# thunlp/ConvDR

Measured on AMD Instinct MI355X. Metric: passages encoded/sec + query x passage IP-scored/sec, 768-d, higher is better.
Workload: dtype bf16

## Files before the change

### convdr_amd/csrc/encoder.hip

```cpp
#include "gemm_launch.hpp"
#include "gemm_ln.hpp"

#include "../../include/convdr_hip.h"

namespace convdr {

struct EncBufs {
  int32_t* status;
  int32_t *tok_id, *tok_pos;
  bf16_t *X, *Q, *K, *Vt, *ctx, *Hm, *cls_b, *cls_ctx, *cls_x, *cls_x1;
  float *Y, *cls_y, *cls_f, *head_y;
  float* slab;
  int64_t ldt;
  size_t total;
};

constexpr int64_t SPLITK_MAX_ROWS = 42 * 128;
constexpr int SPLITK_MAX_SPLIT = 4;
static int64_t g_ffn2_splitk = 1;

static EncBufs enc_plan(const convdr_encoder_config* c, int64_t rows, int B, char* base) {
  EncBufs p;
  size_t o = 0;
  auto take = [&](size_t bytes) { size_t at = o; o = align_up(o + bytes, 256); return (char*)((uintptr_t)base + at); };
  const int H = c->hidden, I = c->intermediate;
  const int64_t rs = rows + 128;
  p.ldt = align_up((size_t)rows + 64, 8);
  p.status = (int32_t*)take(256);
  p.tok_id = (int32_t*)take(rs * 4);
  p.tok_pos = (int32_t*)take(rs * 4);
  p.X = (bf16_t*)take(rs * H * 2);
  p.Q = (bf16_t*)take(rs * H * 2);
  p.K = (bf16_t*)take(rs * H * 2);
  p.Vt = (bf16_t*)take((size_t)H * p.ldt * 2);
  p.ctx = (bf16_t*)take(rs * H * 2);
  p.Hm = (bf16_t*)take(rs * I * 2);
  p.Y = (float*)take(rs * H * 4);
  p.slab = rows <= SPLITK_MAX_ROWS ? (float*)take((size_t)SPLITK_MAX_SPLIT * rs * H * 4) : nullptr;
  const int64_t Bp = B + 128;
  p.cls_b = (bf16_t*)take(Bp * H * 2);
  p.cls_ctx = (bf16_t*)take(Bp * H * 2);
  p.cls_x = (bf16_t*)take(Bp * H * 2);
  p.cls_x1 = (bf16_t*)take(Bp * H * 2);
  p.cls_y = (float*)take(Bp * H * 4);
  p.cls_f = (float*)take(Bp * H * 4);
  p.head_y = (float*)take(Bp * (c->out_dim > 0 ? c->out_dim : 1) * 4);
  p.total = o;
  return p;
}

static int64_t g_fused_ln_max_k = 1 << 30;
static int64_t g_hm_blocked = 1;
static int64_t g_fused_ln_min_rows = 128 * 192;

static bool fused_ln_applies(int64_t rows, int H, int K) {
  return H == 768 && rows >= g_fused_ln_min_rows && K % LN_SLICE == 0 && K <= g_fused_ln_max_k;
}
static int gemm_resid_ln(const bf16_t* W, const bf16_t* Wks, const bf16_t* A, int64_t rows, int H, int K, const float* bias,
                         const bf16_t* R, const float* gamma, const float* beta, float eps, float* Yf, bf16_t* X,
                         const char* name, hipStream_t st, bool a_blocked = false, float* slab = nullptr) {
  if (fused_ln_applies(rows, H, K)) {
    static DeviceOnce attr_done;
    if (attr_done.first())
      CONVDR_CHECK_HIP(
          hipFuncSetAttribute((const void*)k_gemm_resid_ln, hipFuncAttributeMaxDynamicSharedMemorySize, LN_SMEM_BYTES));
    GemmLnArgs a{W, A, rows, K, bias, R, gamma, beta, eps, X,
                 K == 768 ? (unsigned long long*)g_gemm_trace_ln : nullptr, Wks, a_blocked ? 1 : 0, 0};
#ifdef CONVDR_ENABLE_TRACE
    static const int dbg_epi = getenv("CONVDR_DBG_SKIP_EPI") ? atoi(getenv("CONVDR_DBG_SKIP_EPI")) : 0;
    a.dbg_skip_epi = dbg_epi == 1;
#endif
    ProfScope prof(name, st);
    hipLaunchKernelGGL(k_gemm_resid_ln, dim3((unsigned)ceil_div64(rows, TileLN::TL)), dim3(512), LN_SMEM_BYTES, st, a);
    CONVDR_CHECK_LAUNCH("k_gemm_resid_ln");
    return 0;
  }
  GemmArgs g{};
  int ns = 1;
  if (slab && g_ffn2_splitk && H == 768 && K >= 2048 && rows <= SPLITK_MAX_ROWS) {
    const int64_t tiles = ceil_div64(rows, 128) * (H / 128), slots = (int64_t)device_cu_count() * 2;
    for (int c = SPLITK_MAX_SPLIT; c >= 2; c >>= 1)
      if (tiles * c <= slots && K % (c * GEMM_BK) == 0) { ns = c; break; }
  }
  if (ns > 1) {
    g.rows = rows; g.W = W; g.X = A; g.N = H; g.K = K; g.k_split_len = K / ns; g.Cf = slab;
    if (int e = launch_gemm<EPI_SLAB_F32>(g, st, name)) return e;
    ProfScope prof("layernorm", st);
    hipLaunchKernelGGL(k_slab_finish_ln<3>, dim3((unsigned)ceil_div64(rows, 4)), dim3(256), 0, st, slab, ns, rows, bias, R, gamma, beta,
                       eps, X);
    CONVDR_CHECK_LAUNCH("k_slab_finish_ln");
    return 0;
  }
  g.rows = rows; g.W = W; g.X = A; g.N = H; g.K = K; g.bias = bias; g.Cf = Yf; g.R = R;
  if (int e = launch_gemm<EPI_RESID_F32>(g, st, name)) return e;
  ProfScope prof("layernorm", st);
  launch_layernorm_bf16(Yf, rows, H, gamma, beta, eps, X, st);
  CONVDR_CHECK_LAUNCH("k_layernorm");
  return 0;
}

static int check_config(const convdr_encoder_config* c) {
  CONVDR_REQUIRE(c->hidden % 128 == 0 && c->hidden <= 1024, "encoder: hidden must be a multiple of 128, <= 1024 (got %d)",
                 c->hidden);
  CONVDR_REQUIRE(c->heads * 64 == c->hidden, "encoder: head_dim must be 64 (hidden=%d heads=%d)", c->hidden, c->heads);
  CONVDR_REQUIRE(c->intermediate % 64 == 0, "encoder: intermediate %% 64 != 0 (%d)", c->intermediate);
  CONVDR_REQUIRE(c->out_dim == 0 || (c->out_dim % 4 == 0 && c->out_dim <= 1024), "encoder: bad out_dim %d", c->out_dim);
  return 0;
}

int encoder_layer_forward(const convdr_encoder_config* c, const convdr_layer_weights* w, const EncBufs& p,
                          const int32_t* cu, const int32_t* lens, int64_t rows, int B, int max_len, float* lse,
                          bool cls_only, hipStream_t st) {
  const int H = c->hidden, I = c->intermediate;
  GemmArgs g{};
  g.rows = rows;
  g.W = (const bf16_t*)w->wqkv; g.X = p.X; g.N = 3 * H; g.K = H; g.bias = w->bqkv;
  g.Qo = p.Q; g.Ko = p.K; g.Vt = p.Vt; g.H = H; g.ldt = p.ldt;
  const bf16_t *xin = p.X, *ctx = p.ctx;
  bf16_t* x1 = p.X;
  int64_t n = rows;
  const bool blk_on = g_hm_blocked != 0;
  const bool ctx_blocked = blk_on && !cls_only && fused_ln_applies(rows, H, H);
  const bool qk_blocked = blk_on && fused_ln_applies(rows, H, H);
  g.qk_blocked = qk_blocked ? 1 : 0;
  if (!cls_only) {
    if (int e = launch_gemm<EPI_QKV>(g, st, "gemm_qkv")) return e;
    AttnArgs a{p.Q, p.K, p.Vt, p.ldt, cu, lens, H, (int64_t)H, p.ctx, lse, 0.125f, (unsigned long long*)g_attn_trace};
    ProfScope prof("attention", st);
    if (ctx_blocked && qk_blocked) {
      hipLaunchKernelGGL((k_attention_fwd<false, true, true>), dim3((max_len + 127) / 128, c->heads, B), dim3(256), ATT_SMEM_BYTES, st, a);
    } else {
      hipLaunchKernelGGL(k_attention_fwd<false>, dim3((max_len + 127) / 128, c->heads, B), dim3(256), ATT_SMEM_BYTES, st, a);
    }
    CONVDR_CHECK_LAUNCH("k_attention_fwd");
  } else {
    hipLaunchKernelGGL(k_gather_cls, dim3((B + 3) / 4), dim3(256), 0, st, cu, B, H, p.X, (const float*)nullptr, p.cls_x,
                       (float*)nullptr);
    CONVDR_CHECK_LAUNCH("k_gather_cls");
    g.W = (const bf16_t*)w->wqkv + (size_t)H * H; g.bias = w->bqkv + H; g.N = 2 * H; g.third0 = 1;
    if (int e = launch_gemm<EPI_QKV>(g, st, "gemm_qkv")) return e;
    GemmArgs gq{};
    gq.rows = B; gq.W = (const bf16_t*)w->wqkv; gq.X = p.cls_x; gq.N = H; gq.K = H; gq.bias = w->bqkv; gq.Cb = p.Q;
    if (int e = launch_gemm<EPI_BF16>(gq, st, "gemm_qkv")) return e;
    AttnArgs a{p.Q, p.K, p.Vt, p.ldt, cu, lens, H, (int64_t)H, p.cls_ctx, nullptr, 0.125f, nullptr};
    ProfScope prof("attention", st);
    if (qk_blocked) hipLaunchKernelGGL((k_attention_fwd<true, false, true>), dim3(1, c->heads, B), dim3(256), ATT_SMEM_BYTES, st, a);
    else hipLaunchKernelGGL(k_attention_fwd<true>, dim3(1, c->heads, B), dim3(256), ATT_SMEM_BYTES, st, a);
    CONVDR_CHECK_LAUNCH("k_attention_fwd<cls>");
    xin = p.cls_x; ctx = p.cls_ctx; x1 = p.cls_x1; n = B;
  }
  if (int e = gemm_resid_ln((const bf16_t*)w->wo, (const bf16_t*)w->wo_ks, ctx, n, H, H, w->bo, xin, w->ln1_g, w->ln1_b, c->ln_eps, p.Y, x1,
                            "gemm_attn_out", st, ctx_blocked))
    return e;
  GemmArgs g2{};
  g2.rows = n; g2.W = (const bf16_t*)w->w1; g2.X = x1; g2.N = I; g2.K = H; g2.bias = w->b1; g2.Cb = p.Hm;
  const bool blocked = blk_on && !cls_only && fused_ln_applies(n, H, I) && I % 256 == 0 && (I / 256) * ceil_div64(n, 256) >= 192;
  if (blocked) {
    if (int e = launch_gemm<EPI_GELU_BLK>(g2, st, "gemm_ffn1")) return e;
    return gemm_resid_ln((const bf16_t*)w->w2, (const bf16_t*)w->w2_ks, p.Hm, n, H, I, w->b2, x1, w->ln2_g, w->ln2_b, c->ln_eps, p.Y,
                         p.X, "gemm_ffn2", st, true);
  }
  if (int e = launch_gemm<EPI_GELU_BF16>(g2, st, "gemm_ffn1")) return e;
  if (cls_only) {
    g2 = GemmArgs{};
    g2.rows = n; g2.W = (const bf16_t*)w->w2; g2.X = p.Hm; g2.N = H; g2.K = I; g2.bias = w->b2; g2.Cf = p.Y; g2.R = x1;
    return launch_gemm<EPI_RESID_F32>(g2, st, "gemm_ffn2");
  }
  return gemm_resid_ln((const bf16_t*)w->w2, (const bf16_t*)w->w2_ks, p.Hm, n, H, I, w->b2, x1, w->ln2_g, w->ln2_b, c->ln_eps, p.Y, p.X, "gemm_ffn2", st,
                       false, p.slab);
}

}

using namespace convdr;

extern "C" size_t convdr_encoder_workspace_bytes(const convdr_encoder_config* cfg, int64_t rows, int B) {
  return enc_plan(cfg, rows, B, nullptr).total;
}

extern "C" int convdr_cast_f32_bf16(const float* x, void* y, int64_t n, convdr_stream_t stream) {
  CONVDR_REQUIRE(n % 4 == 0, "convdr_cast_f32_bf16: n %% 4 != 0 (%lld)", (long long)n);
  if (n == 0) return 0;
  const int64_t n4 = n / 4;
  const unsigned grid = (unsigned)(ceil_div64(n4, 256) < 4096 ? ceil_div64(n4, 256) : 4096);
  hipLaunchKernelGGL(k_cast_f32_bf16, dim3(grid), dim3(256), 0, (hipStream_t)stream, x, (bf16_t*)y, n4);
  CONVDR_CHECK_LAUNCH("k_cast_f32_bf16");
  return 0;
}

extern "C" int convdr_encoder_forward(const convdr_encoder_config* cfg, const convdr_encoder_weights* w,
                                      const void* input_ids, int ids_are_int32, const int64_t* attention_mask, int B, int L,
                                      const int32_t* cu_seqlens, const int32_t* seq_lens, int64_t rows, int max_len,
                                      void* workspace, size_t workspace_bytes, float* out, convdr_stream_t stream) {
  hipStream_t st = (hipStream_t)stream;
  if (int e = check_config(cfg)) return e;
  CONVDR_REQUIRE(B > 0 && L > 0 && rows > 0 && rows % 8 == 0 && max_len > 0 && max_len <= L,
                 "convdr_encoder_forward: bad sizes B=%d L=%d rows=%lld max_len=%d", B, L, (long long)rows, max_len);
  const EncBufs p = enc_plan(cfg, rows, B, (char*)workspace);
  CONVDR_REQUIRE(workspace_bytes >= p.total, "convdr_encoder_forward: workspace too small (%zu < %zu)", workspace_bytes,
                 p.total);
  const int H = cfg->hidden;
  CONVDR_CHECK_HIP(hipMemset2DAsync(p.Vt + rows, p.ldt * 2, 0, (p.ldt - rows) * 2, H, st));
  CONVDR_CHECK_HIP(hipMemsetAsync(p.status, 0, 256, st));
  hipLaunchKernelGGL(k_seq_pack, dim3((B + 3) / 4), dim3(256), 0, st, input_ids, ids_are_int32, attention_mask, seq_lens, B, L, cu_seqlens,
                     cfg->kind, cfg->pad_idx, cfg->max_pos, cfg->vocab, p.tok_id, p.tok_pos, p.status);
  CONVDR_CHECK_LAUNCH("k_seq_pack");
  {
    ProfScope prof("embed_ln", st);
    hipLaunchKernelGGL(k_embed_ln, dim3((unsigned)ceil_div64(rows, 4)), dim3(256), 0, st, p.tok_id, p.tok_pos, rows, H,
                       w->word_emb, w->pos_emb, w->type_emb, w->emb_ln_g, w->emb_ln_b, cfg->ln_eps, p.X, DropSite{0u, 0u, 1.f});
    CONVDR_CHECK_LAUNCH("k_embed_ln");
  }
  for (int l = 0; l < cfg->layers; ++l) {
    const convdr_layer_weights* lw = &w->layers[l];
    const bool last = l + 1 == cfg->layers;
    if (int e = encoder_layer_forward(cfg, lw, p, cu_seqlens, seq_lens, rows, B, max_len, nullptr, last && !cfg->pool_mean, st))
      return e;
    if (last && cfg->pool_mean) {
      hipLaunchKernelGGL(k_masked_mean, dim3(B), dim3(256), 0, st, p.X, cu_seqlens, seq_lens, H, p.cls_b,
                         cfg->out_dim > 0 ? p.cls_f : out);
      CONVDR_CHECK_LAUNCH("k_masked_mean");
    } else if (last) {
      float* cls_out = cfg->out_dim > 0 ? p.cls_f : out;
      hipLaunchKernelGGL(k_layernorm, dim3((B + 3) / 4), dim3(256), 0, st, p.Y, (int64_t)B, H, lw->ln2_g, lw->ln2_b,
                         cfg->ln_eps, p.cls_b, cls_out);
      CONVDR_CHECK_LAUNCH("k_layernorm(cls)");
    }
  }
  if (cfg->out_dim > 0) {
    GemmArgs g{};
    g.rows = B; g.W = (const bf16_t*)w->head_w; g.X = p.cls_b; g.N = cfg->out_dim; g.K = H; g.bias = w->head_b;
    g.Cf = p.head_y;
    if (int e = launch_gemm<EPI_F32>(g, st, "gemm_head")) return e;
    hipLaunchKernelGGL(k_layernorm, dim3((B + 3) / 4), dim3(256), 0, st, p.head_y, (int64_t)B, cfg->out_dim,
                       w->head_ln_g, w->head_ln_b, cfg->head_ln_eps, (bf16_t*)nullptr, out);
    CONVDR_CHECK_LAUNCH("k_layernorm(head)");
  }
  return 0;
}

extern "C" int convdr_encoder_debug_layout(const convdr_encoder_config* cfg, int64_t rows, int B, int64_t* out) {
  const EncBufs p = enc_plan(cfg, rows, B, nullptr);
  const void* v[13] = {p.tok_id, p.tok_pos, p.X, p.Q, p.K, p.Vt, p.ctx, p.Hm, p.Y, p.cls_b, p.cls_y, p.cls_f, p.head_y};
  for (int i = 0; i < 13; ++i) out[i] = (int64_t)(size_t)v[i];
  out[13] = p.ldt;
  return 0;
}

namespace convdr {
static __global__ void __launch_bounds__(256) k_pack_kslice(const bf16_t* __restrict__ w, int n, int k, bf16_t* __restrict__ out) {
  const int64_t total = (int64_t)n * (k / 8);
  for (int64_t i = (int64_t)blockIdx.x * blockDim.x + threadIdx.x; i < total; i += (int64_t)gridDim.x * blockDim.x) {
    const int c = (int)(i & 3);
    const int64_t sr = i >> 2;
    const int r = (int)(sr % n), s = (int)(sr / n);
    *(uint4*)(out + i * 8) = *(const uint4*)(w + (int64_t)r * k + s * 32 + c * 8);
  }
}
}

extern "C" int convdr_pack_kslice(const void* w_bf16, int n, int k, void* out, convdr_stream_t stream) {
  CONVDR_REQUIRE(n > 0 && k > 0 && k % 32 == 0, "convdr_pack_kslice: bad shape %d x %d", n, k);
  const int64_t total = (int64_t)n * (k / 8);
  hipLaunchKernelGGL(k_pack_kslice, dim3((unsigned)(ceil_div64(total, 256) < 4096 ? ceil_div64(total, 256) : 4096)), dim3(256), 0,
                     (hipStream_t)stream, (const bf16_t*)w_bf16, n, k, (bf16_t*)out);
  CONVDR_CHECK_LAUNCH("k_pack_kslice");
  return 0;
}

extern "C" int convdr_set_option(const char* name, int64_t value) {
  if (strcmp(name, "fused_ln_min_rows") == 0) {
    g_fused_ln_min_rows = value;
    return 0;
  }
  if (strcmp(name, "hm_blocked") == 0) {
    g_hm_blocked = value;
    return 0;
  }
  if (strcmp(name, "gemm_tile_policy") == 0) {
    g_gemm_tile_policy = value;
    return 0;
  }
  if (strcmp(name, "attn_bwd_fused") == 0) {
    g_attn_bwd_fused = value;
    return 0;
  }
  if (strcmp(name, "embed_bwd_deterministic") == 0) {
    g_embed_bwd_det = value;
    return 0;
  }
  if (strcmp(name, "ip_fused_finish") == 0) {
    convdr::g_ip_fused_finish = value;
    return 0;
  }
  if (strcmp(name, "gelu_gp") == 0) {
    g_gelu_gp = value;
    return 0;
  }
  if (strcmp(name, "ffn2_splitk") == 0) {
    g_ffn2_splitk = value;
    return 0;
  }
  if (strcmp(name, "ln_rows") == 0) {
    g_ln_rows = value;
    return 0;
  }
  if (strcmp(name, "ln_bwd_rows") == 0) {
    g_ln_bwd_rows = value;
    return 0;
  }
  if (strcmp(name, "fused_ln_max_k") == 0) {
    g_fused_ln_max_k = value;
    return 0;
  }
  if (strcmp(name, "clock_probe") == 0) {
    g_clock_probe = (void*)(uintptr_t)value;
    g_clock_probe_next = 0;
    return 0;
  }
  if (strcmp(name, "clock_probe_slots") == 0) {
    g_clock_probe_slots = value > 0 ? value : 1;
    return 0;
  }
  if (strcmp(name, "attn_trace") == 0) {
    g_attn_trace = (void*)(uintptr_t)value;
    return 0;
  }
  if (strcmp(name, "gemm_trace_ln") == 0) {
    g_gemm_trace_ln = (void*)(uintptr_t)value;
    return 0;
  }
  if (strcmp(name, "gemm_trace") == 0) {
    g_gemm_trace = (void*)(uintptr_t)value;
    return 0;
  }
  set_error("convdr_set_option: unknown option %s", name);
  return -1;
}
```

Measured before the change: 44800.

## Fold K/V projections into CLS-only last-layer attention via query-weight algebra

```diff
diff --git a/convdr_amd/csrc/cls_fold.hpp b/convdr_amd/csrc/cls_fold.hpp
--- /dev/null
+++ b/convdr_amd/csrc/cls_fold.hpp
@@ -0,0 +1,261 @@
+#pragma once
+#include "gemm_nt.hpp"
+
+namespace convdr {
+
+union Frag8 {
+  bf16x8 v;
+  uint32_t u[4];
+  uint4 q;
+  uint2 d[2];
+};
+
+__device__ __forceinline__ void split_bf16x8(const float* x, Frag8& hi, Frag8& lo) {
+#pragma unroll
+  for (int i = 0; i < 4; ++i) {
+    const uint32_t h = pack_bf16x2(x[2 * i], x[2 * i + 1]);
+    hi.u[i] = h;
+    lo.u[i] = pack_bf16x2(x[2 * i] - __uint_as_float(h << 16), x[2 * i + 1] - __uint_as_float(h & 0xffff0000u));
+  }
+}
+
+constexpr int64_t CLS_FOLD_MIN_ROWS = 16384;
+constexpr int FOLD_ROWS = 64;
+constexpr int FOLD_NC = 128;
+constexpr int FOLD_LDW = FOLD_NC + 4;
+
+static __global__ void __launch_bounds__(256) k_cls_key_fold(const bf16_t* __restrict__ Q, const bf16_t* __restrict__ Wk, int B,
+                                                             int H, float scale, float* __restrict__ U) {
+  __shared__ __attribute__((aligned(16))) bf16_t ws[64 * FOLD_LDW];
+  const int tid = threadIdx.x, lane = tid & 63, wave = tid >> 6, lr = lane & 15, g = lane >> 4;
+  const int h = blockIdx.y, heads = H >> 6;
+  const int b = blockIdx.x * FOLD_ROWS + wave * 16 + lr;
+  const int bc = b < B ? b : B - 1;
+  Frag8 qf[2];
+#pragma unroll
+  for (int ks = 0; ks < 2; ++ks) qf[ks].q = *(const uint4*)(Q + (int64_t)bc * H + h * 64 + ks * 32 + g * 8);
+  const bf16_t* wk = Wk + (int64_t)h * 64 * H;
+  float* up = U + ((int64_t)bc * heads + h) * H;
+  for (int n0 = 0; n0 < H; n0 += FOLD_NC) {
+    __syncthreads();
+#pragma unroll
+    for (int i = 0; i < 4; ++i) {
+      const int idx = i * 256 + tid, r = idx >> 4, c = (idx & 15) * 8;
+      const uint4 v = *(const uint4*)(wk + (int64_t)r * H + n0 + c);
+      *(uint2*)(ws + r * FOLD_LDW + c) = make_uint2(v.x, v.y);
+      *(uint2*)(ws + r * FOLD_LDW + c + 4) = make_uint2(v.z, v.w);
+    }
+    __syncthreads();
+#pragma unroll 2
+    for (int nt = 0; nt < FOLD_NC / 16; ++nt) {
+      f32x4 acc = {0.f, 0.f, 0.f, 0.f};
+#pragma unroll
+      for (int ks = 0; ks < 2; ++ks) {
+        const bf16_t* wp = ws + (ks * 32 + g * 8) * FOLD_LDW + nt * 16 + lr;
+        Frag8 a;
+#pragma unroll
+        for (int i = 0; i < 4; ++i) a.u[i] = (uint32_t)wp[(2 * i) * FOLD_LDW] | ((uint32_t)wp[(2 * i + 1) * FOLD_LDW] << 16);
+        acc = __builtin_amdgcn_mfma_f32_16x16x32_bf16(a.v, qf[ks].v, acc, 0, 0, 0);
+      }
+      if (b < B) *(float4*)(up + n0 + nt * 16 + g * 4) = make_float4(scale * acc[0], scale * acc[1], scale * acc[2], scale * acc[3]);
+    }
+  }
+}
+
+static __global__ void __launch_bounds__(256) k_cls_value_fold(const float* __restrict__ Z, const bf16_t* __restrict__ Wv,
+                                                               const float* __restrict__ bv, int B, int H,
+                                                               bf16_t* __restrict__ ctx) {
+  const int tid = threadIdx.x, lane = tid & 63, wave = tid >> 6, lr = lane & 15, g = lane >> 4;
+  const int h = blockIdx.y, heads = H >> 6;
+  const int b = blockIdx.x * FOLD_ROWS + wave * 16 + lr;
+  const int bc = b < B ? b : B - 1;
+  const float* zp = Z + ((int64_t)bc * heads + h) * H + g * 8;
+  const bf16_t* wv = Wv + ((int64_t)h * 64 + lr) * H + g * 8;
+  f32x4 acc[4];
+#pragma unroll
+  for (int mt = 0; mt < 4; ++mt) acc[mt] = f32x4{0.f, 0.f, 0.f, 0.f};
+  for (int k0 = 0; k0 < H; k0 += 128) {
+    f32x4 z[8];
+#pragma unroll
+    for (int i = 0; i < 4; ++i) {
+      z[2 * i] = __builtin_nontemporal_load((const f32x4*)(zp + k0 + i * 32));
+      z[2 * i + 1] = __builtin_nontemporal_load((const f32x4*)(zp + k0 + i * 32 + 4));
+    }
+#pragma unroll
+    for (int i = 0; i < 4; ++i) {
+      const float x[8] = {z[2 * i][0], z[2 * i][1], z[2 * i][2], z[2 * i][3], z[2 * i + 1][0], z[2 * i + 1][1], z[2 * i + 1][2], z[2 * i + 1][3]};
+      Frag8 zh, zl;
+      split_bf16x8(x, zh, zl);
+#pragma unroll
+      for (int mt = 0; mt < 4; ++mt) {
+        Frag8 a;
+        a.q = *(const uint4*)(wv + (int64_t)mt * 16 * H + k0 + i * 32);
+        acc[mt] = __builtin_amdgcn_mfma_f32_16x16x32_bf16(a.v, zh.v, acc[mt], 0, 0, 0);
+        acc[mt] = __builtin_amdgcn_mfma_f32_16x16x32_bf16(a.v, zl.v, acc[mt], 0, 0, 0);
+      }
+    }
+  }
+  if (b >= B) return;
+#pragma unroll
+  for (int mt = 0; mt < 4; ++mt) {
+    const int j0 = h * 64 + mt * 16 + g * 4;
+    const float4 bias = *(const float4*)(bv + j0);
+    uint2 o;
+    o.x = pack_bf16x2(acc[mt][0] + bias.x, acc[mt][1] + bias.y);
+    o.y = pack_bf16x2(acc[mt][2] + bias.z, acc[mt][3] + bias.w);
+    *(uint2*)(ctx + (int64_t)b * H + j0) = o;
+  }
+}
+
+constexpr int POOL_T = 32;
+template <int HC>
+constexpr int pool_smem_bytes() { return POOL_T * (128 * HC + 4) * 2 + 4 * POOL_T * 16 * 4; }
+
+template <int HC>
+static __global__ void __launch_bounds__(256, HC <= 6 ? 2 : 1) k_cls_pool(const bf16_t* __restrict__ X, const float* __restrict__ U,
+                                                         const int32_t* __restrict__ cu, const int32_t* __restrict__ lens,
+                                                         float* __restrict__ Z) {
+  constexpr int H = 128 * HC, LDX = H + 4, HEADS = 2 * HC, NLD = H / 64, HQ = H / 4, RP = H / 8;
+  extern __shared__ __attribute__((aligned(16))) unsigned char pool_smem[];
+  bf16_t* xs = (bf16_t*)pool_smem;
+  float* sp = (float*)(pool_smem + POOL_T * LDX * 2);
+  const int tid = threadIdx.x, lane = tid & 63, wave = tid >> 6, lr = lane & 15, g = lane >> 4;
+  const int b = blockIdx.x;
+  const int64_t base = cu[b];
+  const int len = lens[b];
+  const int nchunks = (len + POOL_T - 1) / POOL_T;
+
+  u32x4_t pre[NLD];
+  auto fetch = [&](int c) {
+#pragma unroll
+    for (int i = 0; i < NLD; ++i) {
+      const int idx = i * 256 + tid, r = idx / RP, cs = idx % RP, t = c * POOL_T + r;
+      pre[i] = u32x4_t{0u, 0u, 0u, 0u};
+      if (t < len) pre[i] = __builtin_nontemporal_load((const u32x4_t*)(X + (base + t) * H + cs * 8));
+    }
+  };
+  auto stash = [&]() {
+#pragma unroll
+    for (int i = 0; i < NLD; ++i) {
+      const int idx = i * 256 + tid, r = idx / RP, cs = idx % RP;
+      *(uint2*)(xs + r * LDX + cs * 8) = make_uint2(pre[i][0], pre[i][1]);
+      *(uint2*)(xs + r * LDX + cs * 8 + 4) = make_uint2(pre[i][2], pre[i][3]);
+    }
+  };
+  fetch(0);
+
+  Frag8 uh[HC], ul[HC];
+  {
+    const float* up = U + ((int64_t)b * HEADS + (lr < HEADS ? lr : 0)) * H + wave * HQ + g * 8;
+#pragma unroll
+    for (int ks = 0; ks < HC; ++ks) {
+      const f32x4 u0 = __builtin_nontemporal_load((const f32x4*)(up + ks * 32));
+      const f32x4 u1 = __builtin_nontemporal_load((const f32x4*)(up + ks * 32 + 4));
+      const float m = lr < HEADS ? 1.f : 0.f;
+      const float x[8] = {m * u0[0], m * u0[1], m * u0[2], m * u0[3], m * u1[0], m * u1[1], m * u1[2], m * u1[3]};
+      split_bf16x8(x, uh[ks], ul[ks]);
+    }
+  }
+  f32x4 acc[NLD];
+#pragma unroll
+  for (int nt = 0; nt < NLD; ++nt) acc[nt] = f32x4{0.f, 0.f, 0.f, 0.f};
+  float m_run = -INFINITY, l_run = 0.f;
+
+  stash();
+  __syncthreads();
+  for (int c = 0; c < nchunks; ++c) {
+    if (c + 1 < nchunks) fetch(c + 1);
+#pragma unroll
+    for (int mt = 0; mt < 2; ++mt) {
+      f32x4 s = {0.f, 0.f, 0.f, 0.f};
+      const bf16_t* xp = xs + (mt * 16 + lr) * LDX + wave * HQ + g * 8;
+#pragma unroll
+      for (int ks = 0; ks < HC; ++ks) {
+        Frag8 a;
+        a.d[0] = *(const uint2*)(xp + ks * 32);
+        a.d[1] = *(const uint2*)(xp + ks * 32 + 4);
+        s = __builtin_amdgcn_mfma_f32_16x16x32_bf16(a.v, uh[ks].v, s, 0, 0, 0);
+        s = __builtin_amdgcn_mfma_f32_16x16x32_bf16(a.v, ul[ks].v, s, 0, 0, 0);
+      }
+#pragma unroll
+      for (int i = 0; i < 4; ++i) sp[(wave * POOL_T + mt * 16 + g * 4 + i) * 16 + lr] = s[i];
+    }
+    __syncthreads();
+    float sv[8], mx = -INFINITY;
+#pragma unroll
+    for (int j = 0; j < 8; ++j) {
+      const int t = g * 8 + j;
+      float v = sp[t * 16 + lr];
+#pragma unroll
+      for (int w = 1; w < 4; ++w) v += sp[(w * POOL_T + t) * 16 + lr];
+      sv[j] = c * POOL_T + t < len ? v : -INFINITY;
+      mx = fmaxf(mx, sv[j]);
+    }
+    mx = fmaxf(mx, __shfl_xor(mx, 16, 64));
+    mx = fmaxf(mx, __shfl_xor(mx, 32, 64));
+    const float m_new = fmaxf(m_run, mx);
+    const float alpha = __expf(m_run - m_new);
+    float pv[8], ps = 0.f;
+#pragma unroll
+    for (int j = 0; j < 8; ++j) {
+      pv[j] = __expf(sv[j] - m_new);
+      ps += pv[j];
+    }
+    ps += __shfl_xor(ps, 16, 64);
+    ps += __shfl_xor(ps, 32, 64);
+    l_run = l_run * alpha + ps;
+    m_run = m_new;
+    Frag8 ph, pl;
+    split_bf16x8(pv, ph, pl);
+#pragma unroll
+    for (int nt = 0; nt < NLD; ++nt) {
+      const bf16_t* xp = xs + (g * 8) * LDX + wave * HQ + nt * 16 + lr;
+      Frag8 a;
+#pragma unroll
+      for (int i = 0; i < 4; ++i) a.u[i] = (uint32_t)xp[(2 * i) * LDX] | ((uint32_t)xp[(2 * i + 1) * LDX] << 16);
+      acc[nt] *= alpha;
+      acc[nt] = __builtin_amdgcn_mfma_f32_16x16x32_bf16(a.v, ph.v, acc[nt], 0, 0, 0);
+      acc[nt] = __builtin_amdgcn_mfma_f32_16x16x32_bf16(a.v, pl.v, acc[nt], 0, 0, 0);
+    }
+    __syncthreads();
+    if (c + 1 < nchunks) {
+      stash();
+      __syncthreads();
+    }
+  }
+  if (lr < HEADS) {
+    const float inv = 1.f / l_run;
+    float* zp = Z + ((int64_t)b * HEADS + lr) * H + wave * HQ + g * 4;
+#pragma unroll
+    for (int nt = 0; nt < NLD; ++nt)
+      *(float4*)(zp + nt * 16) = make_float4(acc[nt][0] * inv, acc[nt][1] * inv, acc[nt][2] * inv, acc[nt][3] * inv);
+  }
+}
+
+template <int HC>
+static int launch_cls_pool_hc(const bf16_t* X, const float* U, const int32_t* cu, const int32_t* lens, int B, float* Z, hipStream_t st) {
+  static DeviceOnce attr_done;
+  if (attr_done.first())
+    CONVDR_CHECK_HIP(hipFuncSetAttribute((const void*)k_cls_pool<HC>, hipFuncAttributeMaxDynamicSharedMemorySize, pool_smem_bytes<HC>()));
+  hipLaunchKernelGGL(k_cls_pool<HC>, dim3(B), dim3(256), pool_smem_bytes<HC>(), st, X, U, cu, lens, Z);
+  CONVDR_CHECK_LAUNCH("k_cls_pool");
+  return 0;
+}
+
+static int launch_cls_pool(const bf16_t* X, const float* U, const int32_t* cu, const int32_t* lens, int B, int H, float* Z,
+                           hipStream_t st) {
+  switch (H / 128) {
+    case 1: return launch_cls_pool_hc<1>(X, U, cu, lens, B, Z, st);
+    case 2: return launch_cls_pool_hc<2>(X, U, cu, lens, B, Z, st);
+    case 3: return launch_cls_pool_hc<3>(X, U, cu, lens, B, Z, st);
+    case 4: return launch_cls_pool_hc<4>(X, U, cu, lens, B, Z, st);
+    case 5: return launch_cls_pool_hc<5>(X, U, cu, lens, B, Z, st);
+    case 6: return launch_cls_pool_hc<6>(X, U, cu, lens, B, Z, st);
+    case 7: return launch_cls_pool_hc<7>(X, U, cu, lens, B, Z, st);
+    case 8: return launch_cls_pool_hc<8>(X, U, cu, lens, B, Z, st);
+  }
+  set_error("cls fold: hidden %d is not a multiple of 128 <= 1024", H);
+  return -1;
+}
+
+}
diff --git a/convdr_amd/csrc/encoder.hip b/convdr_amd/csrc/encoder.hip
--- a/convdr_amd/csrc/encoder.hip
+++ b/convdr_amd/csrc/encoder.hip
@@ -1,5 +1,6 @@
 #include "gemm_launch.hpp"
 #include "gemm_ln.hpp"
+#include "cls_fold.hpp"
 
 #include "../../include/convdr_hip.h"
 
@@ -52,6 +53,8 @@
 static int64_t g_fused_ln_max_k = 1 << 30;
 static int64_t g_hm_blocked = 1;
 static int64_t g_fused_ln_min_rows = 128 * 192;
+static int64_t g_cls_fold = 1;
+static int64_t g_cls_fold_min_rows = CLS_FOLD_MIN_ROWS;
 
 static bool fused_ln_applies(int64_t rows, int H, int K) {
   return H == 768 && rows >= g_fused_ln_min_rows && K % LN_SLICE == 0 && K <= g_fused_ln_max_k;
@@ -137,16 +140,36 @@
     hipLaunchKernelGGL(k_gather_cls, dim3((B + 3) / 4), dim3(256), 0, st, cu, B, H, p.X, (const float*)nullptr, p.cls_x,
                        (float*)nullptr);
     CONVDR_CHECK_LAUNCH("k_gather_cls");
-    g.W = (const bf16_t*)w->wqkv + (size_t)H * H; g.bias = w->bqkv + H; g.N = 2 * H; g.third0 = 1;
-    if (int e = launch_gemm<EPI_QKV>(g, st, "gemm_qkv")) return e;
     GemmArgs gq{};
     gq.rows = B; gq.W = (const bf16_t*)w->wqkv; gq.X = p.cls_x; gq.N = H; gq.K = H; gq.bias = w->bqkv; gq.Cb = p.Q;
     if (int e = launch_gemm<EPI_BF16>(gq, st, "gemm_qkv")) return e;
-    AttnArgs a{p.Q, p.K, p.Vt, p.ldt, cu, lens, H, (int64_t)H, p.cls_ctx, nullptr, 0.125f, nullptr};
-    ProfScope prof("attention", st);
-    if (qk_blocked) hipLaunchKernelGGL((k_attention_fwd<true, false, true>), dim3(1, c->heads, B), dim3(256), ATT_SMEM_BYTES, st, a);
-    else hipLaunchKernelGGL(k_attention_fwd<true>, dim3(1, c->heads, B), dim3(256), ATT_SMEM_BYTES, st, a);
-    CONVDR_CHECK_LAUNCH("k_attention_fwd<cls>");
+    const size_t fold_bytes = (size_t)B * c->heads * H * sizeof(float);
+    const bool fold = g_cls_fold != 0 && rows >= g_cls_fold_min_rows && fold_bytes <= (size_t)(rows + 128) * H * 2 && fold_bytes <= (size_t)H * p.ldt * 2;
+    if (fold) {
+      float *U = (float*)p.K, *Z = (float*)p.Vt;
+      const dim3 fgrid((unsigned)((B + FOLD_ROWS - 1) / FOLD_ROWS), (unsigned)c->heads);
+      {
+        ProfScope prof("gemm_qkv", st);
+        hipLaunchKernelGGL(k_cls_key_fold, fgrid, dim3(256), 0, st, p.Q, (const bf16_t*)w->wqkv + (size_t)H * H, B, H, 0.125f, U);
+        CONVDR_CHECK_LAUNCH("k_cls_key_fold");
+      }
+      {
+        ProfScope prof("attention", st);
+        if (int e = launch_cls_pool(p.X, U, cu, lens, B, H, Z, st)) return e;
+      }
+      ProfScope prof("gemm_qkv", st);
+      hipLaunchKernelGGL(k_cls_value_fold, fgrid, dim3(256), 0, st, Z, (const bf16_t*)w->wqkv + (size_t)2 * H * H, w->bqkv + 2 * H, B, H,
+                         p.cls_ctx);
+      CONVDR_CHECK_LAUNCH("k_cls_value_fold");
+    } else {
+      g.W = (const bf16_t*)w->wqkv + (size_t)H * H; g.bias = w->bqkv + H; g.N = 2 * H; g.third0 = 1;
+      if (int e = launch_gemm<EPI_QKV>(g, st, "gemm_qkv")) return e;
+      AttnArgs a{p.Q, p.K, p.Vt, p.ldt, cu, lens, H, (int64_t)H, p.cls_ctx, nullptr, 0.125f, nullptr};
+      ProfScope prof("attention", st);
+      if (qk_blocked) hipLaunchKernelGGL((k_attention_fwd<true, false, true>), dim3(1, c->heads, B), dim3(256), ATT_SMEM_BYTES, st, a);
+      else hipLaunchKernelGGL(k_attention_fwd<true>, dim3(1, c->heads, B), dim3(256), ATT_SMEM_BYTES, st, a);
+      CONVDR_CHECK_LAUNCH("k_attention_fwd<cls>");
+    }
     xin = p.cls_x; ctx = p.cls_ctx; x1 = p.cls_x1; n = B;
   }
   if (int e = gemm_resid_ln((const bf16_t*)w->wo, (const bf16_t*)w->wo_ks, ctx, n, H, H, w->bo, xin, w->ln1_g, w->ln1_b, c->ln_eps, p.Y, x1,
@@ -277,6 +300,14 @@
     g_hm_blocked = value;
     return 0;
   }
+  if (strcmp(name, "cls_fold") == 0) {
+    g_cls_fold = value;
+    return 0;
+  }
+  if (strcmp(name, "cls_fold_min_rows") == 0) {
+    g_cls_fold_min_rows = value;
+    return 0;
+  }
   if (strcmp(name, "gemm_tile_policy") == 0) {
     g_gemm_tile_policy = value;
     return 0;
```

Result: no change. 45860, median of 6 (+2.4%).
